# InteractiveComputerGraphics/stark

Measured on AMD Instinct MI355X. Metric: Newton-steps/s, higher is better.
Workload: dtype f64

## Files before the change

stark_amd/csrc/api.cpp:

```cpp
#include <algorithm>
#include <chrono>
#include <cstring>
#include <cstdio>
#include <cstdlib>
#include <string>

#include "dist.hpp"
#include "engine.hpp"
#include "forces.hpp"
#include "../../include/mistark_contact.h"

using namespace mistark;

#define API_BEGIN        \
    if (!ctx) return -1; \
    int _ret = 0;        \
    (void)_ret;          \
    ::mistark::DryScope _dry(ctx->c.dry); \
    try {                \
        if (!ctx->c.dry) (void)hipSetDevice(ctx->c.device);
#define API_END(ret)                   \
    }                                  \
    catch (const std::exception& e)    \
    {                                  \
// ... 1422 lines not shown
{
    API_BEGIN
    const std::string n = name ? name : "";
    if (n == "force_generic") {
        ctx->c.force_generic = value != 0;
        ctx->c.layout_dirty = true;
    }
    else if (n == "generic_contact") ctx->c.generic_contact = value != 0;
    else if (n == "no_eval_prelaunch") ctx->c.no_eval_prelaunch = value != 0;
    else if (n == "no_multi_eval_p") ctx->c.no_multi_eval_p = value != 0;
    else if (n == "no_multi_eval_pgh") ctx->c.no_multi_eval_pgh = value != 0;
    else if (n == "llt_multifrontal") ctx->c.llt_multifrontal = value;
    else if (n == "llt_no_coords") { ctx->c.llt_no_coords = value != 0; ctx->c.llt_mf_pattern_version = 0; }
    else if (n == "generic_inertia") ctx->c.generic_inertia = value != 0;
    else if (n == "contact_closed_min_lanes") ctx->c.contact_closed_min_lanes = value;
    else if (n == "atomic_assembly") ctx->c.atomic_assembly = value != 0;
    else if (n == "spmv_grid_cap") ctx->c.spmv_grid_cap = value;
    else if (n == "spmv_nt") ctx->c.spmv_nt = value;
    else if (n == "custom_rtc") ctx->c.custom_rtc = value;
    else if (n == "custom_timing") ctx->c.custom_timing = value;
    else if (n == "pcg_batch") ctx->c.pcg_batch = value;
    else if (n == "lazy_hessians") ctx->c.lazy_allowed = value != 0;
    else if (n == "lazy_eval") ctx->c.lazy_eval = value != 0;
    else if (n == "no_pattern_overlap") ctx->c.no_pattern_overlap = value != 0;
    else if (n == "no_eval_overlap") ctx->c.no_eval_overlap = value != 0;
    else if (n == "no_eager_assembly") ctx->c.no_eager_assembly = value != 0;
    else if (n == "no_sym_gather") ctx->c.no_sym_gather = value != 0;
    else if (n == "no_split_gather") ctx->c.no_split_gather = value != 0;
    else if (n == "no_bounded_pattern") { ctx->c.no_bounded_pattern = value != 0; ctx->c.part[1].dirty = true; }
    else if (n == "no_grad_gather") { ctx->c.no_grad_gather = value != 0; ctx->c.layout_dirty = true; }

    else if (n == "spmv_variant") ctx->c.spmv_variant = value;
    else if (n == "proj_variant") ctx->c.proj_variant = value;
    else if (n == "no_contact_cache") ctx->c.no_contact_cache = value != 0;
    else if (n == "no_sharded_search") ctx->c.no_sharded_search = value != 0;
    else if (n == "no_row_order") { ctx->c.no_row_order = value != 0; ctx->c.perm_sig.clear(); ctx->c.layout_dirty = true; }
    else if (n == "row_order") { ctx->c.row_order_mode = value; ctx->c.perm_sig.clear(); ctx->c.layout_dirty = true; }
    else if (n == "atomic_projection") ctx->c.atomic_projection = value != 0;
    else if (n == "no_dyn_pool") { ctx->c.no_dyn_pool = value != 0; ctx->c.layout_dirty = true; }
    else if (n == "no_halo_subset") { ctx->c.no_halo_subset = value != 0; ctx->c.cg_mask_pattern = 0; }
    else if (n == "cg_variant") ctx->c.cg_variant = value;
    else if (n == "no_fused_pcg") ctx->c.no_fused_pcg = value != 0;
    else if (n == "spmv_chunk_tiles") {
        if (value < 0 || value > 64) throw Error("spmv_chunk_tiles: 0 (automatic) .. 64");
        ctx->c.spmv_chunk_tiles = value;
        ctx->c.part[0].dirty = true;
    }
    else throw Error("unknown option '" + n + "'");
    API_END(0)
}

int mistark_sync(mistark_ctx* ctx)
{
    API_BEGIN
    MS_CHECK(hipStreamSynchronize(ctx->c.stream));
    API_END(0)
}
int mistark_spmv_bench(mistark_ctx* ctx, int n_launches, double* avg_us)
{
    API_BEGIN
    const double us = spmv_bench(ctx->c, n_launches);
    if (avg_us) *avg_us = us;
    API_END(0)
}

int mistark_spmv_event_overhead(mistark_ctx* ctx, double* avg_ms)
// ... 218 lines not shown
```

stark_amd/csrc/engine.hpp:

```cpp
#pragma once
#include <algorithm>
#include <cstdlib>
#include <hip/hip_runtime.h>

#include <cstdint>
#include <cstdio>
#include <stdexcept>
#include <map>
#include <string>
#include <vector>

#include <memory>

#include "../../include/mistark.h"

#include "potargs.hpp"

namespace mistark {

struct Error : std::runtime_error
{
    using std::runtime_error::runtime_error;
};

// ... 215 lines not shown

    std::vector<DofSet> dof_sets;
    std::vector<Array> arrays;
    std::vector<Potential> pots;
    bool layout_dirty = true;

    int64_t ndofs = 0, nbr = 0;
    DevBuf<double> u, grad, du, r, z, p, q, tmp_a, tmp_b;
    DevBuf<double> p2;
    size_t n_elem_total = 0, hess_total = 0;
    DevBuf<double> elemE, elemH;
    DevBuf<float> elemHf;
    size_t hf_total = 0;
    bool lazy_allowed = true;
    bool lazy_eval = false;
    bool lazy_active = false;
    bool no_grad_gather = false;
    hipStream_t side_stream = nullptr;
    hipEvent_t side_ev[2] = {nullptr, nullptr};
    bool no_pattern_overlap = false;
    hipStream_t aux_stream = nullptr;
    hipEvent_t aux_ev[4] = {nullptr, nullptr, nullptr, nullptr};
    bool no_eval_overlap = false;
    bool no_bounded_pattern = false;
    DevBuf<uint8_t> is_projected, active_blocks;
    bool have_hessians = false;

    BsrPart part[2];
    DevBuf<int32_t> diag_slot[2];
    int spmv_variant = 0;
    int spmv_chunk_tiles = 0;
    DevBuf<unsigned char> sel_desc;
    std::vector<unsigned char> sel_desc_host;
    DevBuf<double> vlong_part;
    DevBuf<double> grad_hot;
    DevBuf<int32_t> hot_rows;
    int n_hot = 0;
    int proj_variant = 0;
    int pcg_batch = 0;
    int spmv_grid_cap = 0;
    int custom_rtc = 1;
    int custom_timing = 0;
    double custom_kernel_us = 0.0;
    int64_t n_rtc_builds = 0, n_rtc_launches = 0;
    double t_rtc_builds = 0.0;
    int spmv_nt = -1;
    bool atomic_assembly = false;
    bool force_generic = false;
    bool generic_inertia = false;
    bool generic_contact = false;
    int contact_closed_min_lanes = -1;
    DevBuf<uint8_t> cub_tmp;
    DevBuf<float> dinv;
    DevBuf<double> dense;
    DevBuf<double> llt_D, llt_S, llt_y;
    DevBuf<int32_t> llt_perm;
    DevBuf<int> llt_info;
    int llt_mb = 0;
    void* llt_mf = nullptr;
    uint64_t llt_mf_pattern_version = 0;
    double llt_mf_gb = 0.0;
    bool llt_no_coords = false;
    int llt_multifrontal = 0;
    int llt_last_path = -1;
    int64_t llt_last_panel_rows = 0, llt_last_panels = 0, llt_last_fronts = 0;
    uint64_t pattern_version = 1, llt_pattern_version = 0;
// ... 526 lines not shown
```

stark_amd/csrc/project.hip:

```cpp
#include "kernels_common.hpp"

namespace mistark {


struct SelDesc
{
    const int32_t* conn;
    const uint32_t* elem_list;
    const int32_t* lrow;
    uint8_t* is_projected;
    uint32_t* list;
    uint32_t* list_e;
    int conn_stride, e_count, NB, counter, first_block, n_own;
    int dof_col[MAX_NB], dof_row_off[MAX_NB];
};
__global__ __launch_bounds__(BLOCK) void k_project_select_multi(const SelDesc* __restrict__ D, int n_desc, const uint8_t* __restrict__ active_blocks, int64_t* __restrict__ counters)
{
    __shared__ int s_k;
    if (threadIdx.x == 0) {
        int k = 0;
        while (k + 1 < n_desc && (int)blockIdx.x >= D[k + 1].first_block) k++;
        s_k = k;
    }
    __syncthreads();
    const SelDesc& d = D[s_k];
    const int le = ((int)blockIdx.x - d.first_block) * BLOCK + threadIdx.x;
    if (le >= d.e_count) return;
    const int e = d.elem_list ? (int)d.elem_list[le] : le;
    if (d.is_projected[le]) return;
    const int32_t* ce = d.conn + (size_t)e * d.conn_stride;
    if (active_blocks) {
        bool touch = false;
        for (int k = 0; k < d.NB; k++) touch = touch || active_blocks[d.dof_row_off[k] + ce[d.dof_col[k]]];
        if (!touch) return;
    }
    d.is_projected[le] = 1;
    const unsigned long long sel = __ballot(1);
    const int lane = threadIdx.x & 63, leader = __ffsll((long long)sel) - 1;
    unsigned long long base = 0;
    if (lane == leader) base = atomicAdd((unsigned long long*)&counters[d.counter], (unsigned long long)__popcll(sel));
    base = ((unsigned long long)(unsigned int)__shfl((int)(base >> 32), leader, 64) << 32) | (unsigned int)__shfl((int)base, leader, 64);
    const unsigned long long idx = base + (unsigned long long)__popcll(sel & ((1ull << lane) - 1ull));
    d.list[idx] = (uint32_t)le;
    d.list_e[idx] = (uint32_t)e;
    bool mine = true;
    if (d.lrow) {
        const int l = d.lrow[d.dof_row_off[0] + ce[d.dof_col[0]]];
        mine = l >= 0 && l < d.n_own;
    }
    const unsigned long long m = __ballot(mine);
// ... 93 lines not shown
                    A[t] = v[c];
                    V[t] = u[c];
                }
            }
        }
    }
    bool bad = false;
    if (lane < n) {
        double l = A[lane * n + lane];
        if (l < eps) {
            bad = true;
            l = (mirroring & 1) ? -l : eps;
        }
        sL[wave][lane] = l;
    }
    const bool changed = __ballot(bad) != 0ull;
    if (lane == 0 && changed) atomicAdd((unsigned long long*)&counters[1], 1ull);
    if (!changed) return;
    for (int t = lane; t < nn; t += 64) {
        const int i = t / n, j = t - i * n;
        double acc = 0.0;
        for (int k = 0; k < n; k++) acc = fma(V[i * n + k] * V[j * n + k], sL[wave][k], acc);
        const int ba = i / 3, ii = i - 3 * ba, bb = j / 3, jj = j - 3 * bb;
        const size_t blk = (size_t)(ba * NB + bb) * n_elem + e;
        double* dst = elemH + (size_t)(ba * NB + bb) * hs + (size_t)pe * 9 + ii * 3 + jj;
        if (vals) {
            const uint32_t slot = slot_of_src[blk];
            if (slot != NO_SRC) atomicAdd(&vals[tile_val_index(slot, ii * 3 + jj)], (float)(acc - *dst));
        }
        *dst = acc;
    }
}

template <int n>
__device__ __forceinline__ double pick(const double (&x)[n], int idx)
{
    double r = 0.0;
#pragma unroll
    for (int i = 0; i < n; i++) r = i == idx ? x[i] : r;
    return r;
}
__device__ __forceinline__ int rr_partner(int m, int r, int i) { return i == m - 1 ? r : (i == r ? m - 1 : (2 * r - i + 2 * (m - 1)) % (m - 1)); }
template <int NB>
struct ProjWaveShared
{
    static constexpr int n = 3 * NB, m = (n + 1) & ~1, W = m, EPW = 64 / W;
    double M[EPW + 1][m * W];
    double2 CS[EPW + 1][m];
    double L[EPW + 1][m];
    double R[64 + W];
};
template <int NB>
__device__ __forceinline__ void project_cols_body(ProjWaveShared<NB>& S, int w, double* __restrict__ elemH, int n_elem, int n_pool, int compact, const uint32_t* __restrict__ list,
                                                  int n_list, double eps, int mirroring, const uint32_t* __restrict__ slot_of_src, float* __restrict__ vals,
                                                  int64_t* __restrict__ counters)
{
    constexpr int n = 3 * NB, nn = n * n, m = (n + 1) & ~1, W = m, EPW = 64 / W;
    const int lane = threadIdx.x & 63;
    const int g = lane / W, c = lane - g * W;
    if (w * EPW >= n_list) return;
    const int li = w * EPW + g;
    const bool elem_ok = g < EPW && li < n_list;
    const bool valid = elem_ok && c < n;
    const int e = elem_ok ? (int)list[li] : 0;
    const int pe = compact ? (elem_ok ? li : 0) : e;
    const size_t hs = (size_t)n_pool * 9;
    const int bb = c / 3, jj = c - 3 * bb;
    double* M = S.M[g];
    double a[n], v[n];
#pragma unroll
    for (int i = 0; i < n; i++) {
        const int ba = i / 3, ii = i - 3 * ba;
        a[i] = valid ? elemH[(size_t)(ba * NB + bb) * hs + (size_t)pe * 9 + ii * 3 + jj] : 0.0;
        v[i] = i == c ? 1.0 : 0.0;
    }
    auto group_sum = [&](double x) {
        S.R[lane] = x;
        double sum = 0.0;
#pragma unroll
        for (int k = 0; k < W; k++) sum += S.R[g * W + k];
        return sum;
    };
    double fro = 0.0;
#pragma unroll
    for (int i = 0; i < n; i++) fro += a[i] * a[i];
    fro = group_sum(fro);
    bool active = elem_ok;
    auto rsqrt_nr = [](double x) {
        double y = __builtin_amdgcn_rsq(x);
        y = y * (1.5 - 0.5 * x * y * y);
        return y * (1.5 - 0.5 * x * y * y);
    };
    auto rcp_nr = [](double x) {
        const double y = __builtin_amdgcn_rcp(x);
        return fma(y, fma(-x, y, 1.0), y);
    };
    auto shfl64 = [](double x, int addr) {
        const int lo = __builtin_amdgcn_ds_bpermute(addr, __double2loint(x)), hi = __builtin_amdgcn_ds_bpermute(addr, __double2hiint(x));
        return __hiloint2double(hi, lo);
    };
    for (int sweep = 0; sweep < 30; sweep++) {
// ... 71 lines not shown
#pragma unroll 1
    for (int i = 0; i < n; i++) {
        double acc = 0.0;
#pragma unroll
        for (int k = 0; k < n; k++) acc = fma(M[i * W + k] * wc[k], S.L[g][k], acc);
        const int ba = i / 3, ii = i - 3 * ba;
        const size_t blk = (size_t)(ba * NB + bb) * n_elem + e;
        double* dst = elemH + (size_t)(ba * NB + bb) * hs + (size_t)pe * 9 + ii * 3 + jj;
        if (vals) {
            const uint32_t slot = slot_of_src[blk];
            if (slot != NO_SRC) atomicAdd(&vals[tile_val_index(slot, ii * 3 + jj)], (float)(acc - *dst));
        }
        *dst = acc;
    }
}

template <int NB>
struct ProjTiShared
{
    static constexpr int n = 3 * (NB - 1), m = (n + 1) & ~1, W = m, EPW = 64 / W;
    double M[EPW + 1][m * W];
    double P[EPW + 1][m * W];
    double2 CS[EPW + 1][m];
    double L[EPW + 1][m];
    double R[64 + W];
};
__device__ __forceinline__ double helmert(int i, int k)
{
    const double s = rsqrt((double)((k + 1) * (k + 2)));
    return i <= k ? s : (i == k + 1 ? -(double)(k + 1) * s : 0.0);
}
template <int NB>
__device__ __forceinline__ void project_ti_body(ProjTiShared<NB>& S, int w, double* __restrict__ elemH, int n_elem, int n_pool, int compact, const uint32_t* __restrict__ list, int n_list,
                                                double eps, int mirroring, const uint32_t* __restrict__ slot_of_src, float* __restrict__ vals, int64_t* __restrict__ counters)
{
    constexpr int n = 3 * (NB - 1), m = (n + 1) & ~1, W = m, EPW = 64 / W;
    const int lane = threadIdx.x & 63;
    const int g = lane / W, c = lane - g * W;
    if (w * EPW >= n_list) return;
    const int li = w * EPW + g;
    const bool elem_ok = g < EPW && li < n_list;
    const bool valid = elem_ok && c < n;
    const int e = elem_ok ? (int)list[li] : 0;
    const int pe = compact ? (elem_ok ? li : 0) : e;
    const size_t hs = (size_t)n_pool * 9;
    double* M = S.M[g];
    double* Pm = S.P[g];
    double a[n], v[n];
    {
        const int ap = valid ? c / 3 : 0, cc = valid ? c - 3 * (c / 3) : 0;
        double qa[NB];
#pragma unroll
        for (int i = 0; i < NB; i++) qa[i] = helmert(i, ap);
        double T[NB][3];
#pragma unroll
        for (int i = 0; i < NB; i++)
#pragma unroll
            for (int ci = 0; ci < 3; ci++) {
                double t = 0.0;
#pragma unroll
                for (int b = 0; b < NB; b++) t += qa[b] * (valid ? elemH[(size_t)(i * NB + b) * hs + (size_t)pe * 9 + ci * 3 + cc] : 0.0);
                T[i][ci] = t;
            }
#pragma unroll
        for (int ip = 0; ip < NB - 1; ip++)
#pragma unroll
            for (int ci = 0; ci < 3; ci++) {
                double t = 0.0;
#pragma unroll
                for (int i = 0; i < NB; i++) t += helmert(i, ip) * T[i][ci];
                a[ip * 3 + ci] = t;
            }
#pragma unroll
        for (int i = 0; i < n; i++) v[i] = i == c ? 1.0 : 0.0;
    }
    auto group_sum = [&](double x) {
        S.R[lane] = x;
        double sum = 0.0;
#pragma unroll
        for (int k = 0; k < W; k++) sum += S.R[g * W + k];
// ... 96 lines not shown
    for (int pass = 0; pass < 2; pass++) {
        const int oc = pass == 0 ? c : n + c;
        if (pass == 0 ? c >= n : c >= 3) continue;
        const int ao = oc / 3, cc = oc - 3 * ao;
        double U[NB - 1][3];
#pragma unroll
        for (int ip = 0; ip < NB - 1; ip++)
#pragma unroll
            for (int ci = 0; ci < 3; ci++) {
                double t = 0.0;
#pragma unroll
                for (int bp = 0; bp < NB - 1; bp++) t += helmert(ao, bp) * Pm[(ip * 3 + ci) * W + (bp * 3 + cc)];
                U[ip][ci] = t;
            }
#pragma unroll 1
        for (int i = 0; i < NB; i++) {
#pragma unroll
            for (int ci = 0; ci < 3; ci++) {
                const int orow = i * 3 + ci;
                if (orow < oc) continue;
                double acc = ci == cc ? null_val / (double)NB : 0.0;
#pragma unroll
                for (int ip = 0; ip < NB - 1; ip++) acc += helmert(i, ip) * U[ip][ci];
#pragma unroll
                for (int side = 0; side < 2; side++) {
                    if (side == 1 && orow == oc) break;
                    const int bi = side == 0 ? i : ao, bj = side == 0 ? ao : i, ii = side == 0 ? ci : cc, jj = side == 0 ? cc : ci;
                    double* dst = elemH + (size_t)(bi * NB + bj) * hs + (size_t)pe * 9 + ii * 3 + jj;
                    if (vals) {
                        const uint32_t slot = slot_of_src[(size_t)(bi * NB + bj) * n_elem + e];
                        if (slot != NO_SRC) atomicAdd(&vals[tile_val_index(slot, ii * 3 + jj)], (float)(acc - *dst));
                    }
                    *dst = acc;
                }
            }
        }
    }
}
template <int NB>
__global__ __launch_bounds__(64) void k_project_eig_ti(double* __restrict__ elemH, int n_elem, int n_pool, int compact, const uint32_t* __restrict__ list, int n_list, double eps,
                                                       int mirroring, const uint32_t* __restrict__ slot_of_src, float* __restrict__ vals, int64_t* __restrict__ counters)
{
    __shared__ ProjTiShared<NB> S;
    project_ti_body<NB>(S, blockIdx.x, elemH, n_elem, n_pool, compact, list, n_list, eps, mirroring, slot_of_src, vals, counters);
}

template <int NB>
__global__ __launch_bounds__(BLOCK) void k_project_eig_cols(double* __restrict__ elemH, int n_elem, int n_pool, int compact, const uint32_t* __restrict__ list, int n_list, double eps,
                                                            int mirroring, const uint32_t* __restrict__ slot_of_src, float* __restrict__ vals, int64_t* __restrict__ counters)
{
    __shared__ ProjWaveShared<NB> S[4];
    const int wave = threadIdx.x >> 6;
    project_cols_body<NB>(S[wave], blockIdx.x * 4 + wave, elemH, n_elem, n_pool, compact, list, n_list, eps, mirroring, slot_of_src, vals, counters);
}
struct ProjDesc
{
    double* H;
    const uint32_t* list;
    const uint32_t* sos;
    float* vals;
    int n_elem, nl, NB, first_wave;
    int n_pool, compact;
    int ti;
};
constexpr int PROJ_BATCH = 40;
struct ProjBatch
{
    ProjDesc d[PROJ_BATCH];
    int n;
};
union ProjWaveSharedAny
{
    ProjWaveShared<1> s1;
    ProjWaveShared<2> s2;
    ProjWaveShared<3> s3;
    ProjWaveShared<4> s4;
    ProjWaveShared<5> s5;
    ProjWaveShared<6> s6;
    ProjTiShared<3> t3;
    ProjTiShared<4> t4;
    __device__ ProjWaveSharedAny() {}
};
__global__ __launch_bounds__(BLOCK) void k_project_eig_multi(ProjBatch B, double eps, int mirroring, int64_t* __restrict__ counters)
{
    __shared__ ProjWaveSharedAny S[4];
    const int wave = threadIdx.x >> 6;
    const int gw = blockIdx.x * 4 + wave;
    int k = 0;
    while (k + 1 < B.n && gw >= B.d[k + 1].first_wave) k++;
    const ProjDesc& D = B.d[k];
    const int w = gw - D.first_wave;
    if (D.ti) {
        if (D.NB == 4) project_ti_body<4>(S[wave].t4, w, D.H, D.n_elem, D.n_pool, D.compact, D.list, D.nl, eps, mirroring, D.sos, D.vals, counters);
        else project_ti_body<3>(S[wave].t3, w, D.H, D.n_elem, D.n_pool, D.compact, D.list, D.nl, eps, mirroring, D.sos, D.vals, counters);
        return;
    }
    switch (D.NB) {
        case 1: project_cols_body<1>(S[wave].s1, w, D.H, D.n_elem, D.n_pool, D.compact, D.list, D.nl, eps, mirroring, D.sos, D.vals, counters); break;
        case 2: project_cols_body<2>(S[wave].s2, w, D.H, D.n_elem, D.n_pool, D.compact, D.list, D.nl, eps, mirroring, D.sos, D.vals, counters); break;
        case 3: project_cols_body<3>(S[wave].s3, w, D.H, D.n_elem, D.n_pool, D.compact, D.list, D.nl, eps, mirroring, D.sos, D.vals, counters); break;
        case 4: project_cols_body<4>(S[wave].s4, w, D.H, D.n_elem, D.n_pool, D.compact, D.list, D.nl, eps, mirroring, D.sos, D.vals, counters); break;
        case 5: project_cols_body<5>(S[wave].s5, w, D.H, D.n_elem, D.n_pool, D.compact, D.list, D.nl, eps, mirroring, D.sos, D.vals, counters); break;
        default: project_cols_body<6>(S[wave].s6, w, D.H, D.n_elem, D.n_pool, D.compact, D.list, D.nl, eps, mirroring, D.sos, D.vals, counters); break;
    }
}

__global__ __launch_bounds__(BLOCK) void k_active_blocks(const double* __restrict__ grad, int64_t nbr, double thr, uint8_t* __restrict__ active, int64_t* __restrict__ counters,
                                                        const int32_t* __restrict__ lrow, int n_own)
{
    const int64_t r = (int64_t)blockIdx.x * BLOCK + threadIdx.x;
    const bool in = r < nbr;
    const double m = in ? fmax(fabs(grad[3 * r]), fmax(fabs(grad[3 * r + 1]), fabs(grad[3 * r + 2]))) : 0.0;
    const bool act = !in || m >= thr;
    if (in) active[r] = act ? 1 : 0;
    const bool own = in && (!lrow || (lrow[r] >= 0 && lrow[r] < n_own));
    __shared__ int s_cnt[BLOCK / 64];
    const unsigned long long inactive = __ballot(!act && own);
    if ((threadIdx.x & 63) == 0) s_cnt[threadIdx.x >> 6] = __popcll(inactive);
    __syncthreads();
    if (threadIdx.x == 0) {
        const int n = s_cnt[0] + s_cnt[1] + s_cnt[2] + s_cnt[3];
        if (n) atomicAdd((unsigned long long*)&counters[2], (unsigned long long)n);
    }
}

struct MarkDesc
{
    const uint32_t* list;
    const uint32_t* slot_of_src;
    uint8_t* dirty;
    const double* Hc;
    float* hf;
    int nl, NB, n_key, n_pool_c, n_pool_f;
    int first_block;
};
constexpr int MARK_BATCH = 16;
// ... 17 lines not shown
    const int nn = NB * NB;
    if (t >= (int64_t)nl * nn) return;
    const int li = (int)(t / nn), ab = (int)(t - (int64_t)li * nn), a = ab / NB, b = ab - a * NB;
    const uint32_t le = list[li];
    const uint32_t slot = slot_of_src[(size_t)ab * n_key + le];
    if (!hf) {
        if (slot != NO_SRC) dirty[slot] = 1;
        return;
    }
    if (a > b) return;
    const double* src = Hc + ((size_t)ab * n_pool_c + li) * 9;
    float* dst = hf + ((size_t)tet_pair_index(a, b) * n_pool_f + le) * 9;
    bool diff = false;
#pragma unroll
    for (int k = 0; k < 9; k++) {
        const float f = (float)src[k];
        if (dst[k] != f) {
            dst[k] = f;
            diff = true;
        }
    }
    if (!diff) return;
    if (slot != NO_SRC) dirty[slot] = 1;
    if (a != b) {
        const uint32_t slot_t = slot_of_src[(size_t)(b * NB + a) * n_key + le];
        if (slot_t != NO_SRC) dirty[slot_t] = 1;
    }
}

static void project_select(Context& c, const uint8_t* active_host, bool by_gradient, double threshold)
{
    const int np = (int)c.pots.size();
    if (np + 4 > 128) throw Error("project: too many potentials");
    c.counters.ensure(128);
    fill_async(c.stream, c.counters.p, 0, 128 * sizeof(int64_t));
    const uint8_t* act = nullptr;
    const int32_t* lrow = c.world > 1 ? c.sh.lrow.p : nullptr;
    if (by_gradient) {
        hipLaunchKernelGGL(k_active_blocks, dim3(grid_for(c.nbr)), dim3(BLOCK), 0, c.stream, c.grad.p, c.nbr, threshold, c.active_blocks.p, c.counters.p, lrow, (int)c.sh.n_own);
        act = c.active_blocks.p;
    } else if (active_host) {
        MS_CHECK(hipMemcpyAsync(c.active_blocks.p, active_host, (size_t)c.nbr, hipMemcpyHostToDevice, c.stream));
        act = c.active_blocks.p;
    }
    c.proj_list.ensure(2 * std::max<size_t>(c.n_elem_total, 1));
    uint32_t* list_e_base = c.proj_list.p + std::max<size_t>(c.n_elem_total, 1);
    c.sel_desc_host.resize((size_t)np * sizeof(SelDesc));
    SelDesc* desc_h = reinterpret_cast<SelDesc*>(c.sel_desc_host.data());
    int n_desc = 0;
    int n_blocks = 0;
    for (int pi = 0; pi < np; pi++) {
        Potential& P = c.pots[pi];
        if (P.args.e_count == 0) continue;
        SelDesc d{};
        d.conn = P.args.conn;
        d.elem_list = P.args.elem_list;
        d.lrow = lrow;
        d.n_own = (int)c.sh.n_own;
        d.is_projected = c.is_projected.p + P.e_off;
        d.list = c.proj_list.p + P.e_off;
        d.list_e = list_e_base + P.e_off;
        d.conn_stride = P.args.conn_stride;
        d.e_count = P.args.e_count;
        d.NB = P.NB;
        d.counter = 4 + pi;
        d.first_block = n_blocks;
        for (int k = 0; k < MAX_NB; k++) {
            d.dof_col[k] = P.args.dof_col[k];
            d.dof_row_off[k] = P.args.dof_row_off[k];
        }
        n_blocks += (P.args.e_count + BLOCK - 1) / BLOCK;
        desc_h[n_desc++] = d;
    }
    if (n_desc > 0) {
        c.sel_desc.ensure((size_t)n_desc * sizeof(SelDesc));
        MS_CHECK(hipMemcpyAsync(c.sel_desc.p, desc_h, (size_t)n_desc * sizeof(SelDesc), hipMemcpyHostToDevice, c.stream));
        hipLaunchKernelGGL(k_project_select_multi, dim3(n_blocks), dim3(BLOCK), 0, c.stream, (const SelDesc*)c.sel_desc.p, n_desc, act, c.counters.p);
    }
}
static void project_selected(Context& c, const int64_t* h, double eps, int mirroring)
{
    const int np = (int)c.pots.size();
    uint32_t* list_e_base = c.proj_list.p + std::max<size_t>(c.n_elem_total, 1);
    struct Mark
    {
        int pot;
        const uint32_t* list;
        int nl;
        const double* Hc;
        int n_pool_c;
    };
    std::vector<Mark> marks;
    bool mark_part[2] = {false, false};
    if (c.proj_variant & 4) mirroring |= 2;
    constexpr int SHORT_LIST = 4096;
    ProjBatch batch;
    batch.n = 0;
    int batch_waves = 0;
    auto flush = [&]() {
        if (batch.n == 0) return;
        hipLaunchKernelGGL(k_project_eig_multi, dim3((batch_waves + 3) / 4), dim3(BLOCK), 0, c.stream, batch, eps, mirroring, c.counters.p);
        batch.n = 0;
        batch_waves = 0;
    };
    for (int pi = 0; pi < np; pi++) {
        Potential& P = c.pots[pi];
        const int nl = (int)h[4 + pi];
        if (nl == 0) continue;
        hipStream_t stream = c.stream;
        double* H = c.elemH.p + P.h_off;
        const uint32_t* list = c.proj_list.p + P.e_off;
        const uint32_t* sos = c.part[P.part].slot_of_src.p + P.kp_off;
        const int n_key = P.n_key;
        int n_pool = P.n_key, compact = 0;
        if (c.lazy_active && P.lazy_capable) {
            n_pool = (nl + 63) / 64 * 64;
            H = c.elemH.p + P.h_off;
            compact = 1;
            launch_tet_closed_list(c, P, list_e_base + P.e_off, nl, H, n_pool);
        }
        float* vals = (c.matrix_current || (c.static_assembled && P.part == 0)) ? c.part[P.part].vals.p : nullptr;
        if (vals && !c.atomic_projection) {
            marks.push_back(Mark{pi, list, nl, compact ? H : (const double*)nullptr, n_pool});
            mark_part[P.part] = true;
            vals = nullptr;
        }
        const dim3 g((nl + 3) / 4), b(BLOCK);
        if (!(c.proj_variant & 1) && P.NB <= 6) {
            const int epw = 64 / ((3 * P.NB + 1) & ~1);
            const bool ti = P.ti_projection && !(c.proj_variant & 8) && (P.NB == 3 || P.NB == 4);
            if (nl <= SHORT_LIST && !(c.proj_variant & 2)) {
                if (batch.n == PROJ_BATCH) flush();
                const int epw_b = ti ? 64 / ((3 * (P.NB - 1) + 1) & ~1) : epw;
                batch.d[batch.n++] = ProjDesc{H, list, sos, vals, n_key, nl, P.NB, batch_waves, n_pool, compact, ti ? 1 : 0};
                batch_waves += (nl + epw_b - 1) / epw_b;
                continue;
            }
            if (ti) {
                const int epw_ti = 64 / ((3 * (P.NB - 1) + 1) & ~1);
                const dim3 grid_ti((nl + epw_ti - 1) / epw_ti), b_ti(64);
                if (P.NB == 4) hipLaunchKernelGGL((k_project_eig_ti<4>), grid_ti, b_ti, 0, stream, H, n_key, n_pool, compact, list, nl, eps, mirroring, sos, vals, c.counters.p);
                else hipLaunchKernelGGL((k_project_eig_ti<3>), grid_ti, b_ti, 0, stream, H, n_key, n_pool, compact, list, nl, eps, mirroring, sos, vals, c.counters.p);
                continue;
            }
            const dim3 grid(((nl + epw - 1) / epw + 3) / 4);
            switch (P.NB) {
                case 1: hipLaunchKernelGGL((k_project_eig_cols<1>), grid, b, 0, stream, H, n_key, n_pool, compact, list, nl, eps, mirroring, sos, vals, c.counters.p); break;
                case 2: hipLaunchKernelGGL((k_project_eig_cols<2>), grid, b, 0, stream, H, n_key, n_pool, compact, list, nl, eps, mirroring, sos, vals, c.counters.p); break;
                case 3: hipLaunchKernelGGL((k_project_eig_cols<3>), grid, b, 0, stream, H, n_key, n_pool, compact, list, nl, eps, mirroring, sos, vals, c.counters.p); break;
                case 4: hipLaunchKernelGGL((k_project_eig_cols<4>), grid, b, 0, stream, H, n_key, n_pool, compact, list, nl, eps, mirroring, sos, vals, c.counters.p); break;
                case 5: hipLaunchKernelGGL((k_project_eig_cols<5>), grid, b, 0, stream, H, n_key, n_pool, compact, list, nl, eps, mirroring, sos, vals, c.counters.p); break;
                default: hipLaunchKernelGGL((k_project_eig_cols<6>), grid, b, 0, stream, H, n_key, n_pool, compact, list, nl, eps, mirroring, sos, vals, c.counters.p); break;
            }
            continue;
        }
        switch (P.NB) {
            case 1: hipLaunchKernelGGL((k_project_eig<1>), g, b, 0, stream, H, n_key, n_pool, compact, list, nl, eps, mirroring, sos, vals, c.counters.p); break;
            case 2: hipLaunchKernelGGL((k_project_eig<2>), g, b, 0, stream, H, n_key, n_pool, compact, list, nl, eps, mirroring, sos, vals, c.counters.p); break;
            case 3: hipLaunchKernelGGL((k_project_eig<3>), g, b, 0, stream, H, n_key, n_pool, compact, list, nl, eps, mirroring, sos, vals, c.counters.p); break;
            case 4: hipLaunchKernelGGL((k_project_eig<4>), g, b, 0, stream, H, n_key, n_pool, compact, list, nl, eps, mirroring, sos, vals, c.counters.p); break;
            case 5: hipLaunchKernelGGL((k_project_eig<5>), g, b, 0, stream, H, n_key, n_pool, compact, list, nl, eps, mirroring, sos, vals, c.counters.p); break;
            case 6: hipLaunchKernelGGL((k_project_eig<6>), g, b, 0, stream, H, n_key, n_pool, compact, list, nl, eps, mirroring, sos, vals, c.counters.p); break;
            case 7: hipLaunchKernelGGL((k_project_eig<7>), g, b, 0, stream, H, n_key, n_pool, compact, list, nl, eps, mirroring, sos, vals, c.counters.p); break;
            case 8: hipLaunchKernelGGL((k_project_eig<8>), g, b, 0, stream, H, n_key, n_pool, compact, list, nl, eps, mirroring, sos, vals, c.counters.p); break;
            default: throw Error("project: unsupported block count");
        }
    }
    flush();
    if (marks.empty()) return;
    for (int part = 0; part < 2; part++)
        if (mark_part[part]) {
            BsrPart& m = c.part[part];
            const size_t n_pos = (size_t)std::max<int64_t>(m.ntiles * 64, m.nnzb) + 4;
            if (m.slot_dirty.cap < n_pos) {
                m.slot_dirty.ensure(n_pos);
                MS_CHECK(hipMemsetAsync(m.slot_dirty.p, 0, m.slot_dirty.cap, c.stream));
            }
        }
    MarkBatch mb;
    mb.n = 0;
    int blocks = 0;
    auto flush_marks = [&]() {
        if (mb.n > 0) hipLaunchKernelGGL(k_proj_mark, dim3(blocks), dim3(BLOCK), 0, c.stream, mb);
        mb.n = 0;
        blocks = 0;
    };
    for (const Mark& k : marks) {
        Potential& P = c.pots[(size_t)k.pot];
        BsrPart& m = c.part[P.part];
        const bool lazy = k.Hc != nullptr;
        if (k.nl <= 0) continue;
        if (mb.n == MARK_BATCH) flush_marks();
        mb.d[mb.n++] = MarkDesc{k.list, (const uint32_t*)(m.slot_of_src.p + P.kp_off), m.slot_dirty.p, k.Hc, lazy ? c.elemHf.p + P.hf_off : (float*)nullptr, k.nl, P.NB, P.n_key,
                                k.n_pool_c, P.n_pool_f, blocks};
        blocks += grid_for((int64_t)k.nl * P.NB * P.NB);
    }
    flush_marks();
    for (int part = 0; part < 2; part++)
        if (mark_part[part]) {
            BsrPart& m = c.part[part];
            gather_part(c, part, m.slot_dirty.p);
            fill_async(c.stream, m.slot_dirty.p, 0, ((size_t)std::max<int64_t>(m.ntiles * 64, m.nnzb) + 3) & ~(size_t)3);
        }
}
void project(Context& c, double eps, int mirroring, const uint8_t* active_host, bool by_gradient, double threshold, int* all_active, int64_t* n_projected_now,
             int64_t* n_changed_now)
{
    if (c.static_assembled) MS_CHECK(hipStreamWaitEvent(c.stream, c.aux_ev[2], 0));
    ensure_pattern(c);
    if (!c.have_hessians) throw Error("project: no element Hessians (call eval with MISTARK_EVAL_P_G_H first)");
    project_select(c, active_host, by_gradient, threshold);
    int64_t h[128];
    fetch(c, h, c.counters.p, sizeof(h));
    int64_t n_inactive = h[2], n_selected = h[3];
    if (c.world > 1) {
        double mine[2] = {(double)h[2], (double)h[3]}, all[2 * 64];
        shard_allgather_scalars(c, mine, 2, all);
        n_inactive = n_selected = 0;
        for (int r = 0; r < c.world; r++) {
            n_inactive += (int64_t)all[2 * r];
            n_selected += (int64_t)all[2 * r + 1];
        }
    }
    project_selected(c, h, eps, mirroring);
    c.n_projected_total += n_selected;
    if (n_projected_now) *n_projected_now = n_selected;
    if (n_changed_now) {
        int64_t h2[2];
        fetch(c, h2, c.counters.p, sizeof(h2));
        *n_changed_now = h2[1];
    }
    if (all_active) *all_active = by_gradient ? (n_inactive == 0) : (active_host == nullptr);
}


}
```

Measured before the change: 215.3.

## Fuse projection dirty-slot marking into eigen kernels and double-buffer counters

The projection eigen kernels now set the slot_dirty flags (and refresh lazy float Hessian copies) in their own epilogue, so the separate mark kernel launch is skipped on the ordered path. Projection counters are double-buffered, and the select kernel zeroes the next buffer, which removes a memset per call. The selection descriptor upload is skipped when the bytes are unchanged. The cost is extra slot lookups inside the eigen kernels and more complex routing logic.

```diff
diff --git a/stark_amd/csrc/api.cpp b/stark_amd/csrc/api.cpp
--- a/stark_amd/csrc/api.cpp
+++ b/stark_amd/csrc/api.cpp
@@ -1478,6 +1478,7 @@
 
     else if (n == "spmv_variant") ctx->c.spmv_variant = value;
     else if (n == "proj_variant") ctx->c.proj_variant = value;
+    else if (n == "proj_epilogue_marks") ctx->c.proj_epilogue_marks = value;
     else if (n == "no_contact_cache") ctx->c.no_contact_cache = value != 0;
     else if (n == "no_sharded_search") ctx->c.no_sharded_search = value != 0;
     else if (n == "no_row_order") { ctx->c.no_row_order = value != 0; ctx->c.perm_sig.clear(); ctx->c.layout_dirty = true; }
diff --git a/stark_amd/csrc/engine.hpp b/stark_amd/csrc/engine.hpp
--- a/stark_amd/csrc/engine.hpp
+++ b/stark_amd/csrc/engine.hpp
@@ -271,6 +271,12 @@
     int spmv_chunk_tiles = 0;
     DevBuf<unsigned char> sel_desc;
     std::vector<unsigned char> sel_desc_host;
+    std::vector<unsigned char> sel_desc_sent;
+    DevBuf<int64_t> proj_counters;
+    int proj_cnt_cur = 0;
+    bool proj_cnt_clean[2] = {false, false};
+    int64_t* proj_cnt = nullptr;
+    int proj_epilogue_marks = 1;
     DevBuf<double> vlong_part;
     DevBuf<double> grad_hot;
     DevBuf<int32_t> hot_rows;
diff --git a/stark_amd/csrc/project.hip b/stark_amd/csrc/project.hip
--- a/stark_amd/csrc/project.hip
+++ b/stark_amd/csrc/project.hip
@@ -14,8 +14,10 @@
     int conn_stride, e_count, NB, counter, first_block, n_own;
     int dof_col[MAX_NB], dof_row_off[MAX_NB];
 };
-__global__ __launch_bounds__(BLOCK) void k_project_select_multi(const SelDesc* __restrict__ D, int n_desc, const uint8_t* __restrict__ active_blocks, int64_t* __restrict__ counters)
-{
+__global__ __launch_bounds__(BLOCK) void k_project_select_multi(const SelDesc* __restrict__ D, int n_desc, const uint8_t* __restrict__ active_blocks, int64_t* __restrict__ counters,
+                                                               int64_t* __restrict__ clear_next)
+{
+    if (clear_next && blockIdx.x == 0 && threadIdx.x < 128) clear_next[threadIdx.x] = 0;
     __shared__ int s_k;
     if (threadIdx.x == 0) {
         int k = 0;
@@ -175,6 +177,20 @@
     }
 }
 
+struct ProjMarks
+{
+    uint8_t* dirty;
+    float* hf;
+    int n_pool_f;
+};
+template <int NB, int W>
+__device__ __forceinline__ void flag_selected(const ProjMarks& mk, const uint32_t* __restrict__ slot_of_src, int n_elem, int e, int c)
+{
+    for (int ab = c; ab < NB * NB; ab += W) {
+        const uint32_t slot = slot_of_src[(size_t)ab * n_elem + e];
+        if (slot != NO_SRC) mk.dirty[slot] = 1;
+    }
+}
 template <int n>
 __device__ __forceinline__ double pick(const double (&x)[n], int idx)
 {
@@ -196,7 +212,7 @@
 template <int NB>
 __device__ __forceinline__ void project_cols_body(ProjWaveShared<NB>& S, int w, double* __restrict__ elemH, int n_elem, int n_pool, int compact, const uint32_t* __restrict__ list,
                                                   int n_list, double eps, int mirroring, const uint32_t* __restrict__ slot_of_src, float* __restrict__ vals,
-                                                  int64_t* __restrict__ counters)
+                                                  int64_t* __restrict__ counters, const ProjMarks mk = ProjMarks{nullptr, nullptr, 0})
 {
     constexpr int n = 3 * NB, nn = n * n, m = (n + 1) & ~1, W = m, EPW = 64 / W;
     const int lane = threadIdx.x & 63;
@@ -210,6 +226,7 @@
     const size_t hs = (size_t)n_pool * 9;
     const int bb = c / 3, jj = c - 3 * bb;
     double* M = S.M[g];
+    if (mk.dirty && !mk.hf && elem_ok) flag_selected<NB, W>(mk, slot_of_src, n_elem, e, c);
     double a[n], v[n];
 #pragma unroll
     for (int i = 0; i < n; i++) {
@@ -347,7 +364,8 @@
 }
 template <int NB>
 __device__ __forceinline__ void project_ti_body(ProjTiShared<NB>& S, int w, double* __restrict__ elemH, int n_elem, int n_pool, int compact, const uint32_t* __restrict__ list, int n_list,
-                                                double eps, int mirroring, const uint32_t* __restrict__ slot_of_src, float* __restrict__ vals, int64_t* __restrict__ counters)
+                                                double eps, int mirroring, const uint32_t* __restrict__ slot_of_src, float* __restrict__ vals, int64_t* __restrict__ counters,
+                                                const ProjMarks mk = ProjMarks{nullptr, nullptr, 0})
 {
     constexpr int n = 3 * (NB - 1), m = (n + 1) & ~1, W = m, EPW = 64 / W;
     const int lane = threadIdx.x & 63;
@@ -361,6 +379,7 @@
     const size_t hs = (size_t)n_pool * 9;
     double* M = S.M[g];
     double* Pm = S.P[g];
+    if (mk.dirty && !mk.hf && elem_ok) flag_selected<NB, W>(mk, slot_of_src, n_elem, e, c);
     double a[n], v[n];
     {
         const int ap = valid ? c / 3 : 0, cc = valid ? c - 3 * (c / 3) : 0;
@@ -523,6 +542,19 @@
                         if (slot != NO_SRC) atomicAdd(&vals[tile_val_index(slot, ii * 3 + jj)], (float)(acc - *dst));
                     }
                     *dst = acc;
+                    if (mk.hf && bi <= bj) {
+                        const float f = (float)acc;
+                        float* df = mk.hf + ((size_t)tet_pair_index(bi, bj) * mk.n_pool_f + e) * 9 + ii * 3 + jj;
+                        if (*df != f) {
+                            *df = f;
+                            const uint32_t slot = slot_of_src[(size_t)(bi * NB + bj) * n_elem + e];
+                            if (slot != NO_SRC) mk.dirty[slot] = 1;
+                            if (bi != bj) {
+                                const uint32_t slot_t = slot_of_src[(size_t)(bj * NB + bi) * n_elem + e];
+                                if (slot_t != NO_SRC) mk.dirty[slot_t] = 1;
+                            }
+                        }
+                    }
                 }
             }
         }
@@ -530,19 +562,21 @@
 }
 template <int NB>
 __global__ __launch_bounds__(64) void k_project_eig_ti(double* __restrict__ elemH, int n_elem, int n_pool, int compact, const uint32_t* __restrict__ list, int n_list, double eps,
-                                                       int mirroring, const uint32_t* __restrict__ slot_of_src, float* __restrict__ vals, int64_t* __restrict__ counters)
+                                                       int mirroring, const uint32_t* __restrict__ slot_of_src, float* __restrict__ vals, int64_t* __restrict__ counters,
+                                                       ProjMarks mk)
 {
     __shared__ ProjTiShared<NB> S;
-    project_ti_body<NB>(S, blockIdx.x, elemH, n_elem, n_pool, compact, list, n_list, eps, mirroring, slot_of_src, vals, counters);
+    project_ti_body<NB>(S, blockIdx.x, elemH, n_elem, n_pool, compact, list, n_list, eps, mirroring, slot_of_src, vals, counters, mk);
 }
 
 template <int NB>
 __global__ __launch_bounds__(BLOCK) void k_project_eig_cols(double* __restrict__ elemH, int n_elem, int n_pool, int compact, const uint32_t* __restrict__ list, int n_list, double eps,
-                                                            int mirroring, const uint32_t* __restrict__ slot_of_src, float* __restrict__ vals, int64_t* __restrict__ counters)
+                                                            int mirroring, const uint32_t* __restrict__ slot_of_src, float* __restrict__ vals, int64_t* __restrict__ counters,
+                                                            ProjMarks mk)
 {
     __shared__ ProjWaveShared<NB> S[4];
     const int wave = threadIdx.x >> 6;
-    project_cols_body<NB>(S[wave], blockIdx.x * 4 + wave, elemH, n_elem, n_pool, compact, list, n_list, eps, mirroring, slot_of_src, vals, counters);
+    project_cols_body<NB>(S[wave], blockIdx.x * 4 + wave, elemH, n_elem, n_pool, compact, list, n_list, eps, mirroring, slot_of_src, vals, counters, mk);
 }
 struct ProjDesc
 {
@@ -553,6 +587,7 @@
     int n_elem, nl, NB, first_wave;
     int n_pool, compact;
     int ti;
+    ProjMarks mk;
 };
 constexpr int PROJ_BATCH = 40;
 struct ProjBatch
@@ -582,17 +617,17 @@
     const ProjDesc& D = B.d[k];
     const int w = gw - D.first_wave;
     if (D.ti) {
-        if (D.NB == 4) project_ti_body<4>(S[wave].t4, w, D.H, D.n_elem, D.n_pool, D.compact, D.list, D.nl, eps, mirroring, D.sos, D.vals, counters);
-        else project_ti_body<3>(S[wave].t3, w, D.H, D.n_elem, D.n_pool, D.compact, D.list, D.nl, eps, mirroring, D.sos, D.vals, counters);
+        if (D.NB == 4) project_ti_body<4>(S[wave].t4, w, D.H, D.n_elem, D.n_pool, D.compact, D.list, D.nl, eps, mirroring, D.sos, D.vals, counters, D.mk);
+        else project_ti_body<3>(S[wave].t3, w, D.H, D.n_elem, D.n_pool, D.compact, D.list, D.nl, eps, mirroring, D.sos, D.vals, counters, D.mk);
         return;
     }
     switch (D.NB) {
-        case 1: project_cols_body<1>(S[wave].s1, w, D.H, D.n_elem, D.n_pool, D.compact, D.list, D.nl, eps, mirroring, D.sos, D.vals, counters); break;
-        case 2: project_cols_body<2>(S[wave].s2, w, D.H, D.n_elem, D.n_pool, D.compact, D.list, D.nl, eps, mirroring, D.sos, D.vals, counters); break;
-        case 3: project_cols_body<3>(S[wave].s3, w, D.H, D.n_elem, D.n_pool, D.compact, D.list, D.nl, eps, mirroring, D.sos, D.vals, counters); break;
-        case 4: project_cols_body<4>(S[wave].s4, w, D.H, D.n_elem, D.n_pool, D.compact, D.list, D.nl, eps, mirroring, D.sos, D.vals, counters); break;
-        case 5: project_cols_body<5>(S[wave].s5, w, D.H, D.n_elem, D.n_pool, D.compact, D.list, D.nl, eps, mirroring, D.sos, D.vals, counters); break;
-        default: project_cols_body<6>(S[wave].s6, w, D.H, D.n_elem, D.n_pool, D.compact, D.list, D.nl, eps, mirroring, D.sos, D.vals, counters); break;
+        case 1: project_cols_body<1>(S[wave].s1, w, D.H, D.n_elem, D.n_pool, D.compact, D.list, D.nl, eps, mirroring, D.sos, D.vals, counters, D.mk); break;
+        case 2: project_cols_body<2>(S[wave].s2, w, D.H, D.n_elem, D.n_pool, D.compact, D.list, D.nl, eps, mirroring, D.sos, D.vals, counters, D.mk); break;
+        case 3: project_cols_body<3>(S[wave].s3, w, D.H, D.n_elem, D.n_pool, D.compact, D.list, D.nl, eps, mirroring, D.sos, D.vals, counters, D.mk); break;
+        case 4: project_cols_body<4>(S[wave].s4, w, D.H, D.n_elem, D.n_pool, D.compact, D.list, D.nl, eps, mirroring, D.sos, D.vals, counters, D.mk); break;
+        case 5: project_cols_body<5>(S[wave].s5, w, D.H, D.n_elem, D.n_pool, D.compact, D.list, D.nl, eps, mirroring, D.sos, D.vals, counters, D.mk); break;
+        default: project_cols_body<6>(S[wave].s6, w, D.H, D.n_elem, D.n_pool, D.compact, D.list, D.nl, eps, mirroring, D.sos, D.vals, counters, D.mk); break;
     }
 }
 
@@ -676,12 +711,20 @@
 {
     const int np = (int)c.pots.size();
     if (np + 4 > 128) throw Error("project: too many potentials");
-    c.counters.ensure(128);
-    fill_async(c.stream, c.counters.p, 0, 128 * sizeof(int64_t));
+    if (c.proj_counters.cap < 256) {
+        c.proj_counters.ensure(256);
+        c.proj_cnt_clean[0] = c.proj_cnt_clean[1] = false;
+    }
+    const int cur = c.proj_cnt_cur ^= 1;
+    c.proj_cnt = c.proj_counters.p + 128 * cur;
+    int64_t* const cnt = c.proj_cnt;
+    int64_t* const cnt_next = c.proj_counters.p + 128 * (cur ^ 1);
+    if (!c.proj_cnt_clean[cur]) fill_async(c.stream, cnt, 0, 128 * sizeof(int64_t));
+    c.proj_cnt_clean[cur] = false;
     const uint8_t* act = nullptr;
     const int32_t* lrow = c.world > 1 ? c.sh.lrow.p : nullptr;
     if (by_gradient) {
-        hipLaunchKernelGGL(k_active_blocks, dim3(grid_for(c.nbr)), dim3(BLOCK), 0, c.stream, c.grad.p, c.nbr, threshold, c.active_blocks.p, c.counters.p, lrow, (int)c.sh.n_own);
+        hipLaunchKernelGGL(k_active_blocks, dim3(grid_for(c.nbr)), dim3(BLOCK), 0, c.stream, c.grad.p, c.nbr, threshold, c.active_blocks.p, cnt, lrow, (int)c.sh.n_own);
         act = c.active_blocks.p;
     } else if (active_host) {
         MS_CHECK(hipMemcpyAsync(c.active_blocks.p, active_host, (size_t)c.nbr, hipMemcpyHostToDevice, c.stream));
@@ -717,10 +760,54 @@
         desc_h[n_desc++] = d;
     }
     if (n_desc > 0) {
-        c.sel_desc.ensure((size_t)n_desc * sizeof(SelDesc));
-        MS_CHECK(hipMemcpyAsync(c.sel_desc.p, desc_h, (size_t)n_desc * sizeof(SelDesc), hipMemcpyHostToDevice, c.stream));
-        hipLaunchKernelGGL(k_project_select_multi, dim3(n_blocks), dim3(BLOCK), 0, c.stream, (const SelDesc*)c.sel_desc.p, n_desc, act, c.counters.p);
-    }
+        const size_t bytes = (size_t)n_desc * sizeof(SelDesc);
+        if (c.sel_desc.cap < bytes) {
+            c.sel_desc.ensure(bytes);
+            c.sel_desc_sent.clear();
+        }
+        if (c.sel_desc_sent.size() != bytes || std::memcmp(c.sel_desc_sent.data(), desc_h, bytes) != 0) {
+            c.sel_desc_sent.assign(c.sel_desc_host.data(), c.sel_desc_host.data() + bytes);
+            MS_CHECK(hipMemcpyAsync(c.sel_desc.p, c.sel_desc_sent.data(), bytes, hipMemcpyHostToDevice, c.stream));
+        }
+        hipLaunchKernelGGL(k_project_select_multi, dim3(n_blocks), dim3(BLOCK), 0, c.stream, (const SelDesc*)c.sel_desc.p, n_desc, act, cnt, cnt_next);
+        c.proj_cnt_clean[cur ^ 1] = true;
+    }
+}
+constexpr int SHORT_LIST = 4096;
+static void ensure_slot_dirty(Context& c, int part)
+{
+    BsrPart& m = c.part[part];
+    const size_t n_pos = (size_t)std::max<int64_t>(m.ntiles * 64, m.nnzb) + 4;
+    if (m.slot_dirty.cap < n_pos) {
+        m.slot_dirty.ensure(n_pos);
+        MS_CHECK(hipMemsetAsync(m.slot_dirty.p, 0, m.slot_dirty.cap, c.stream));
+    }
+}
+struct ProjRoute
+{
+    bool reg;
+    bool ti;
+    bool lazy;
+    bool patched;
+    bool ordered;
+    bool epilogue;
+};
+static ProjRoute proj_route(const Context& c, const Potential& P)
+{
+    ProjRoute r;
+    r.reg = !(c.proj_variant & 1) && P.NB <= 6;
+    r.ti = r.reg && P.ti_projection && !(c.proj_variant & 8) && (P.NB == 3 || P.NB == 4);
+    r.lazy = c.lazy_active && P.lazy_capable;
+    r.patched = c.matrix_current || (c.static_assembled && P.part == 0);
+    r.ordered = r.patched && !c.atomic_projection;
+    r.epilogue = r.ordered && c.proj_epilogue_marks != 0 && c.world == 1 && r.reg && (!r.lazy || r.ti);
+    return r;
+}
+static ProjMarks proj_marks(Context& c, const Potential& P, const ProjRoute& r)
+{
+    if (!r.epilogue) return ProjMarks{nullptr, nullptr, 0};
+    ensure_slot_dirty(c, P.part);
+    return ProjMarks{c.part[P.part].slot_dirty.p, r.lazy ? c.elemHf.p + P.hf_off : (float*)nullptr, P.n_pool_f};
 }
 static void project_selected(Context& c, const int64_t* h, double eps, int mirroring)
 {
@@ -737,13 +824,12 @@
     std::vector<Mark> marks;
     bool mark_part[2] = {false, false};
     if (c.proj_variant & 4) mirroring |= 2;
-    constexpr int SHORT_LIST = 4096;
     ProjBatch batch;
     batch.n = 0;
     int batch_waves = 0;
     auto flush = [&]() {
         if (batch.n == 0) return;
-        hipLaunchKernelGGL(k_project_eig_multi, dim3((batch_waves + 3) / 4), dim3(BLOCK), 0, c.stream, batch, eps, mirroring, c.counters.p);
+        hipLaunchKernelGGL(k_project_eig_multi, dim3((batch_waves + 3) / 4), dim3(BLOCK), 0, c.stream, batch, eps, mirroring, c.proj_cnt);
         batch.n = 0;
         batch_waves = 0;
     };
@@ -757,70 +843,66 @@
         const uint32_t* sos = c.part[P.part].slot_of_src.p + P.kp_off;
         const int n_key = P.n_key;
         int n_pool = P.n_key, compact = 0;
-        if (c.lazy_active && P.lazy_capable) {
+        const ProjRoute r = proj_route(c, P);
+        if (r.lazy) {
             n_pool = (nl + 63) / 64 * 64;
             H = c.elemH.p + P.h_off;
             compact = 1;
             launch_tet_closed_list(c, P, list_e_base + P.e_off, nl, H, n_pool);
         }
-        float* vals = (c.matrix_current || (c.static_assembled && P.part == 0)) ? c.part[P.part].vals.p : nullptr;
-        if (vals && !c.atomic_projection) {
-            marks.push_back(Mark{pi, list, nl, compact ? H : (const double*)nullptr, n_pool});
+        float* vals = r.patched ? c.part[P.part].vals.p : nullptr;
+        ProjMarks mk{nullptr, nullptr, 0};
+        if (r.ordered) {
+            if (r.epilogue) mk = proj_marks(c, P, r);
+            else marks.push_back(Mark{pi, list, nl, compact ? H : (const double*)nullptr, n_pool});
             mark_part[P.part] = true;
             vals = nullptr;
         }
         const dim3 g((nl + 3) / 4), b(BLOCK);
-        if (!(c.proj_variant & 1) && P.NB <= 6) {
+        if (r.reg) {
             const int epw = 64 / ((3 * P.NB + 1) & ~1);
-            const bool ti = P.ti_projection && !(c.proj_variant & 8) && (P.NB == 3 || P.NB == 4);
+            const bool ti = r.ti;
             if (nl <= SHORT_LIST && !(c.proj_variant & 2)) {
                 if (batch.n == PROJ_BATCH) flush();
                 const int epw_b = ti ? 64 / ((3 * (P.NB - 1) + 1) & ~1) : epw;
-                batch.d[batch.n++] = ProjDesc{H, list, sos, vals, n_key, nl, P.NB, batch_waves, n_pool, compact, ti ? 1 : 0};
+                batch.d[batch.n++] = ProjDesc{H, list, sos, vals, n_key, nl, P.NB, batch_waves, n_pool, compact, ti ? 1 : 0, mk};
                 batch_waves += (nl + epw_b - 1) / epw_b;
                 continue;
             }
             if (ti) {
                 const int epw_ti = 64 / ((3 * (P.NB - 1) + 1) & ~1);
                 const dim3 grid_ti((nl + epw_ti - 1) / epw_ti), b_ti(64);
-                if (P.NB == 4) hipLaunchKernelGGL((k_project_eig_ti<4>), grid_ti, b_ti, 0, stream, H, n_key, n_pool, compact, list, nl, eps, mirroring, sos, vals, c.counters.p);
-                else hipLaunchKernelGGL((k_project_eig_ti<3>), grid_ti, b_ti, 0, stream, H, n_key, n_pool, compact, list, nl, eps, mirroring, sos, vals, c.counters.p);
+                if (P.NB == 4) hipLaunchKernelGGL((k_project_eig_ti<4>), grid_ti, b_ti, 0, stream, H, n_key, n_pool, compact, list, nl, eps, mirroring, sos, vals, c.proj_cnt, mk);
+                else hipLaunchKernelGGL((k_project_eig_ti<3>), grid_ti, b_ti, 0, stream, H, n_key, n_pool, compact, list, nl, eps, mirroring, sos, vals, c.proj_cnt, mk);
                 continue;
             }
             const dim3 grid(((nl + epw - 1) / epw + 3) / 4);
             switch (P.NB) {
-                case 1: hipLaunchKernelGGL((k_project_eig_cols<1>), grid, b, 0, stream, H, n_key, n_pool, compact, list, nl, eps, mirroring, sos, vals, c.counters.p); break;
-                case 2: hipLaunchKernelGGL((k_project_eig_cols<2>), grid, b, 0, stream, H, n_key, n_pool, compact, list, nl, eps, mirroring, sos, vals, c.counters.p); break;
-                case 3: hipLaunchKernelGGL((k_project_eig_cols<3>), grid, b, 0, stream, H, n_key, n_pool, compact, list, nl, eps, mirroring, sos, vals, c.counters.p); break;
-                case 4: hipLaunchKernelGGL((k_project_eig_cols<4>), grid, b, 0, stream, H, n_key, n_pool, compact, list, nl, eps, mirroring, sos, vals, c.counters.p); break;
-                case 5: hipLaunchKernelGGL((k_project_eig_cols<5>), grid, b, 0, stream, H, n_key, n_pool, compact, list, nl, eps, mirroring, sos, vals, c.counters.p); break;
-                default: hipLaunchKernelGGL((k_project_eig_cols<6>), grid, b, 0, stream, H, n_key, n_pool, compact, list, nl, eps, mirroring, sos, vals, c.counters.p); break;
+                case 1: hipLaunchKernelGGL((k_project_eig_cols<1>), grid, b, 0, stream, H, n_key, n_pool, compact, list, nl, eps, mirroring, sos, vals, c.proj_cnt, mk); break;
+                case 2: hipLaunchKernelGGL((k_project_eig_cols<2>), grid, b, 0, stream, H, n_key, n_pool, compact, list, nl, eps, mirroring, sos, vals, c.proj_cnt, mk); break;
+                case 3: hipLaunchKernelGGL((k_project_eig_cols<3>), grid, b, 0, stream, H, n_key, n_pool, compact, list, nl, eps, mirroring, sos, vals, c.proj_cnt, mk); break;
+                case 4: hipLaunchKernelGGL((k_project_eig_cols<4>), grid, b, 0, stream, H, n_key, n_pool, compact, list, nl, eps, mirroring, sos, vals, c.proj_cnt, mk); break;
+                case 5: hipLaunchKernelGGL((k_project_eig_cols<5>), grid, b, 0, stream, H, n_key, n_pool, compact, list, nl, eps, mirroring, sos, vals, c.proj_cnt, mk); break;
+                default: hipLaunchKernelGGL((k_project_eig_cols<6>), grid, b, 0, stream, H, n_key, n_pool, compact, list, nl, eps, mirroring, sos, vals, c.proj_cnt, mk); break;
             }
             continue;
         }
         switch (P.NB) {
-            case 1: hipLaunchKernelGGL((k_project_eig<1>), g, b, 0, stream, H, n_key, n_pool, compact, list, nl, eps, mirroring, sos, vals, c.counters.p); break;
-            case 2: hipLaunchKernelGGL((k_project_eig<2>), g, b, 0, stream, H, n_key, n_pool, compact, list, nl, eps, mirroring, sos, vals, c.counters.p); break;
-            case 3: hipLaunchKernelGGL((k_project_eig<3>), g, b, 0, stream, H, n_key, n_pool, compact, list, nl, eps, mirroring, sos, vals, c.counters.p); break;
-            case 4: hipLaunchKernelGGL((k_project_eig<4>), g, b, 0, stream, H, n_key, n_pool, compact, list, nl, eps, mirroring, sos, vals, c.counters.p); break;
-            case 5: hipLaunchKernelGGL((k_project_eig<5>), g, b, 0, stream, H, n_key, n_pool, compact, list, nl, eps, mirroring, sos, vals, c.counters.p); break;
-            case 6: hipLaunchKernelGGL((k_project_eig<6>), g, b, 0, stream, H, n_key, n_pool, compact, list, nl, eps, mirroring, sos, vals, c.counters.p); break;
-            case 7: hipLaunchKernelGGL((k_project_eig<7>), g, b, 0, stream, H, n_key, n_pool, compact, list, nl, eps, mirroring, sos, vals, c.counters.p); break;
-            case 8: hipLaunchKernelGGL((k_project_eig<8>), g, b, 0, stream, H, n_key, n_pool, compact, list, nl, eps, mirroring, sos, vals, c.counters.p); break;
+            case 1: hipLaunchKernelGGL((k_project_eig<1>), g, b, 0, stream, H, n_key, n_pool, compact, list, nl, eps, mirroring, sos, vals, c.proj_cnt); break;
+            case 2: hipLaunchKernelGGL((k_project_eig<2>), g, b, 0, stream, H, n_key, n_pool, compact, list, nl, eps, mirroring, sos, vals, c.proj_cnt); break;
+            case 3: hipLaunchKernelGGL((k_project_eig<3>), g, b, 0, stream, H, n_key, n_pool, compact, list, nl, eps, mirroring, sos, vals, c.proj_cnt); break;
+            case 4: hipLaunchKernelGGL((k_project_eig<4>), g, b, 0, stream, H, n_key, n_pool, compact, list, nl, eps, mirroring, sos, vals, c.proj_cnt); break;
+            case 5: hipLaunchKernelGGL((k_project_eig<5>), g, b, 0, stream, H, n_key, n_pool, compact, list, nl, eps, mirroring, sos, vals, c.proj_cnt); break;
+            case 6: hipLaunchKernelGGL((k_project_eig<6>), g, b, 0, stream, H, n_key, n_pool, compact, list, nl, eps, mirroring, sos, vals, c.proj_cnt); break;
+            case 7: hipLaunchKernelGGL((k_project_eig<7>), g, b, 0, stream, H, n_key, n_pool, compact, list, nl, eps, mirroring, sos, vals, c.proj_cnt); break;
+            case 8: hipLaunchKernelGGL((k_project_eig<8>), g, b, 0, stream, H, n_key, n_pool, compact, list, nl, eps, mirroring, sos, vals, c.proj_cnt); break;
             default: throw Error("project: unsupported block count");
         }
     }
     flush();
-    if (marks.empty()) return;
+    if (!mark_part[0] && !mark_part[1]) return;
     for (int part = 0; part < 2; part++)
-        if (mark_part[part]) {
-            BsrPart& m = c.part[part];
-            const size_t n_pos = (size_t)std::max<int64_t>(m.ntiles * 64, m.nnzb) + 4;
-            if (m.slot_dirty.cap < n_pos) {
-                m.slot_dirty.ensure(n_pos);
-                MS_CHECK(hipMemsetAsync(m.slot_dirty.p, 0, m.slot_dirty.cap, c.stream));
-            }
-        }
+        if (mark_part[part]) ensure_slot_dirty(c, part);
     MarkBatch mb;
     mb.n = 0;
     int blocks = 0;
@@ -855,7 +937,7 @@
     if (!c.have_hessians) throw Error("project: no element Hessians (call eval with MISTARK_EVAL_P_G_H first)");
     project_select(c, active_host, by_gradient, threshold);
     int64_t h[128];
-    fetch(c, h, c.counters.p, sizeof(h));
+    fetch(c, h, c.proj_cnt, sizeof(h));
     int64_t n_inactive = h[2], n_selected = h[3];
     if (c.world > 1) {
         double mine[2] = {(double)h[2], (double)h[3]}, all[2 * 64];
@@ -871,7 +953,7 @@
     if (n_projected_now) *n_projected_now = n_selected;
     if (n_changed_now) {
         int64_t h2[2];
-        fetch(c, h2, c.counters.p, sizeof(h2));
+        fetch(c, h2, c.proj_cnt, sizeof(h2));
         *n_changed_now = h2[1];
     }
     if (all_active) *all_active = by_gradient ? (n_inactive == 0) : (active_host == nullptr);
```

New measurement: 213.8. No clear change (-0.7%).
